# musaru/Fall_Multimodal

Measured on AMD Instinct MI355X. Metric: clips/sec (fwd+bwd) 3-stream Fall3, B=256, 1/2/4/8 GPUs; top-1 acc parity, higher is better.
Workload: dtype bf16x3; 1 GPU; fall3_3stream_coco_mmpose_V18_S6_B256_per_gpu; global_batch=256, seq_len=30, parallelism=dp1, joints=18, imu_axes=6, classes=11, hip_graph=False, ranks=1

## Files before the change

fall_multimodal_amd/_lib.py:

```python
from __future__ import annotations

import ctypes
import os

import torch

HERE = os.path.dirname(os.path.abspath(__file__))
LIB_PATH = os.environ.get("F3_LIB") or os.path.join(HERE, "libfall3.so")

EXPORTS = (
    "f3_net_create", "f3_net_destroy", "f3_net_num_entries", "f3_net_entry", "f3_net_param_count",
    "f3_net_buffer_count", "f3_net_counter_count", "f3_net_workspace_bytes", "f3_net_forward",
    "f3_net_loss", "f3_net_backward", "f3_rmsprop_step", "f3_conv_forward", "f3_status_string",
    "f3_net_debug_tensor", "f3_conv_backward_data", "f3_conv_backward_weight", "f3_conv_wgrad_packed", "f3_split_x3cat",
    "f3_conv_forward_x3cat", "f3_conv_backward_data_x3cat", "f3_conv_backward_weight_x3cat", "f3_conv_step_x3cat", "f3_graph_mix_forward",
    "f3_graph_mix_backward", "f3_graph_mix_forward_ex", "f3_graph_mix_backward_ex", "f3_gcn_dgrad_mix_x3",
    "f3_gcn_fwd_mix_x3",
    "f3_net_backward_phase",
    "f3_net_grad_split", "f3_net_wait_phase1", "f3_net_backward_rmsprop", "f3_net_fused_rmsprop", "f3_net_precision", "f3_net_status",
    "f3_targcn_create", "f3_targcn_destroy", "f3_targcn_num_entries", "f3_targcn_entry", "f3_targcn_param_count",
    "f3_targcn_buffer_count", "f3_targcn_workspace_bytes", "f3_targcn_forward", "f3_targcn_backward", "f3_targcn_stage_times", "f3_targcn_status", "f3_net_sensor_times", "f3_soft_ce",
    "f3_sktr_create", "f3_sktr_destroy", "f3_sktr_num_entries", "f3_sktr_entry", "f3_sktr_param_count",
    "f3_sktr_buffer_count", "f3_sktr_counter_count", "f3_sktr_workspace_bytes", "f3_sktr_forward", "f3_sktr_backward",
    "f3_musa_create", "f3_musa_destroy", "f3_musa_num_entries", "f3_musa_entry", "f3_musa_param_count",
    "f3_musa_buffer_count", "f3_musa_counter_count", "f3_musa_workspace_bytes", "f3_musa_forward", "f3_musa_backward",
    "f3_musa_guards",
    "f3_dwconv_t_forward", "f3_pointwise_conv", "f3_rgb_scratch_floats", "f3_rgb_forward", "f3_rgb_backward",
    "f3_optim_scalars_bytes", "f3_optim_step", "f3_optim_step_ranges", "f3_net_backward_optim", "f3_net_entry_nograd",
    "f3_metrics_bytes", "f3_metrics_reset", "f3_metrics_update", "f3_segment_norms_scratch_bytes", "f3_segment_norms",
    "f3_soft_ce_ex", "f3_net_loss_ex", "f3_grad_accumulate",
)

F3_OK, F3_EINVAL, F3_EBATCH, F3_EHIP, F3_ESTATE, F3_EDEVICE = 0, 1001, 1002, 1003, 1004, 1005
ENTRY_PARAM, ENTRY_BUFFER, ENTRY_COUNTER = 0, 1, 2
OPT_RMSPROP, OPT_SGD, OPT_ADAM, OPT_ADAMW = 0, 1, 2, 3
OPT_MAX_SKIP = 4
METRICS_MAXK, METRICS_MAXC = 8, 64


class F3OptimConfig(ctypes.Structure):
# ... 65 lines not shown
        "f3_metrics_update": (I, [P, P, P, P, P, I, I, ctypes.POINTER(I), I, P]),
        "f3_segment_norms_scratch_bytes": (I64, [I64, I]),
        "f3_segment_norms": (I, [P, P, P, I, P, P, I64, ctypes.c_double, P]),
        "f3_soft_ce_ex": (I, [P, P, P, I, I, F, P, P, P]),
        "f3_net_loss_ex": (I, [P, I, P, P, F, P, P, P]),
        "f3_grad_accumulate": (I, [P, P, I64, P, P]),
        "f3_conv_forward": (I, [P, P, P, P, P, I, I, I, I, I, I, I, I, I, P]),
        "f3_status_string": (ctypes.c_char_p, [I]),
        "f3_net_debug_tensor": (P, [P, I, P, I, I, ctypes.c_char_p]),
        "f3_conv_backward_data": (I, [P, P, P, P, I, I, I, I, I, I, I, I, I, P]),
        "f3_conv_backward_weight": (I, [P, P, P, P, I, I, I, I, I, I, I, I, I, P]),
        "f3_conv_wgrad_packed": (I, [P, P, P, ctypes.c_longlong, I, I, I, I, I, I, I, I, P]),
        "f3_split_x3cat": (I, [P, P, ctypes.c_int64, I, P]),
        "f3_conv_forward_x3cat": (I, [P, P, P, P, P, I, I, I, I, I, I, I, I, P]),
        "f3_conv_backward_data_x3cat": (I, [P, P, P, P, I, I, I, I, I, I, I, I, P]),
        "f3_conv_backward_weight_x3cat": (I, [P, P, P, P, I, I, I, I, I, I, I, I, P]),
        "f3_conv_step_x3cat": (I, [I, P, P, P, P, P, P, P, P, P, P, F, P, P, I, I, I, I, I, P]),
        "f3_graph_mix_forward": (I, [P, P, P, I, I, I, I, P]),
        "f3_graph_mix_backward": (I, [P, P, P, P, P, I, I, I, I, P]),
        "f3_graph_mix_forward_ex": (I, [P, P, P, I, I, I, I, I, P]),
        "f3_graph_mix_backward_ex": (I, [P, P, P, P, P, I, I, I, I, I, P]),
        "f3_gcn_dgrad_mix_x3": (I, [P, P, P, P, P, P, P, I, I, I, I, I, I, I, P]),
        "f3_gcn_fwd_mix_x3": (I, [P, P, P, P, P, P, P, P, P, I, I, I, I, I, P]),
        "f3_targcn_create": (I, [ctypes.POINTER(F3TargcnConfig), ctypes.POINTER(P)]),
        "f3_targcn_destroy": (None, [P]),
        "f3_targcn_num_entries": (I, [P]),
        "f3_targcn_entry": (I, [P, I, ctypes.POINTER(ctypes.c_char_p), ctypes.POINTER(I), ctypes.POINTER(I),
                                ctypes.POINTER(I64), ctypes.POINTER(I64)]),
        "f3_targcn_param_count": (I64, [P]),
        "f3_targcn_buffer_count": (I64, [P]),
        "f3_targcn_workspace_bytes": (I64, [P, I]),
        "f3_targcn_stage_times": (I, [P, I, P]),
        "f3_targcn_status": (I, [P, I]),
        "f3_net_sensor_times": (I, [P, I, P]),
        "f3_targcn_forward": (I, [P, I, P, P, P, P, P, P]),
        "f3_targcn_backward": (I, [P, I, P, P, P, P, P, P]),
        "f3_soft_ce": (I, [P, P, I, I, P, P, P]),
        "f3_sktr_create": (I, [ctypes.POINTER(F3SktrConfig), ctypes.POINTER(P)]),
        "f3_sktr_destroy": (None, [P]),
        "f3_sktr_num_entries": (I, [P]),
        "f3_sktr_entry": (I, [P, I, ctypes.POINTER(ctypes.c_char_p), ctypes.POINTER(I), ctypes.POINTER(I),
                              ctypes.POINTER(I64), ctypes.POINTER(I64)]),
        "f3_sktr_param_count": (I64, [P]),
        "f3_sktr_buffer_count": (I64, [P]),
        "f3_sktr_counter_count": (I64, [P]),
        "f3_sktr_workspace_bytes": (I64, [P, I]),
# ... 49 lines not shown
```

fall_multimodal_amd/csrc/gcn_fwd.hip:

```cpp
#include "igemm.h"
#include "layers.h"

#include <algorithm>
#include <cstdlib>
#include <type_traits>

namespace f3 {

constexpr int GF_THREADS = 512;
constexpr int GF_VMAX = 18, GF_K = 3, GF_CIN = 64, GF_KC = GF_K * GF_CIN;
constexpr int GF_BM = 32, GF_KS = 2 * GF_KC / 32;
constexpr int GF_XD = 7, GF_NXB = GF_XD + 1;
constexpr int GF_RING = GF_BM * GF_NXB;
constexpr int GF_ZP = GF_BM * 4 * GF_KC / 16 / GF_THREADS;

template <int WN>
struct GfLds {
  static constexpr int NT = 64 * WN;
  static constexpr int ABUF = GF_BM * GF_KC * 2 * 2;
  static constexpr int OTS = NT + 4;
  static constexpr int X_OFF = 2 * ABUF;
  static constexpr int OT_OFF = X_OFF + GF_RING * GF_CIN * 4;
  static constexpr int BV_OFF = OT_OFF + GF_BM * OTS * 4;
  static constexpr int RED_OFF = BV_OFF + GF_VMAX * NT * 4;
  static constexpr int BYTES = RED_OFF + 2 * 2 * NT * 4;
  static constexpr int PIECES = GF_BM * NT * 4 / 16 / GF_THREADS;
};

typedef __bf16 gf_bf16x4 __attribute__((ext_vector_type(4)));
typedef unsigned gf_u32x4 __attribute__((ext_vector_type(4)));

F3_DEV void gf_a_split(float t, __bf16& hi, __bf16& lo) {
  const float h = __uint_as_float(__float_as_uint(t) & 0xffff0000u);
  hi = __builtin_bit_cast(__bf16, (unsigned short)(__float_as_uint(h) >> 16));
  lo = (__bf16)(t - h);
}

F3_DEV float gf_atil(const float* A, int K, int V, int wk, int v) {
  if (wk >= K * V || v >= V) return 0.f;
  const int w = wk / K, k = wk - w * K;
  return A[(k * V + v) * V + w];
}

F3_DEV f32x4 gf_mfma_x3m(bf16x8 ah, bf16x8 al, bf16x8 bh, bf16x8 bl, f32x4 c) {
  c = mfma_bf16x(al, bh, c);
  c = mfma_bf16x(ah, bl, c);
  return mfma_bf16x(ah, bh, c);
}

template <int WN>
__global__ __launch_bounds__(GF_THREADS) void gcn_fwd_mix_x3_kernel(GcnFwdMixArgs a, int per_wg) {
  using L = GfLds<WN>;
  constexpr int NT = L::NT, OTS = L::OTS, KS = GF_KS, K = GF_K, CIN = GF_CIN, PIECES = L::PIECES;
  constexpr int OPS = 1 + GF_ZP + PIECES;
  constexpr int NSTEADY = GF_ZP + OPS * (GF_XD - 2);
  static_assert(L::BYTES <= 160 * 1024 && NSTEADY < 64 && GF_ZP * GF_THREADS * 16 == L::ABUF, "gcn_fwd LDS / vmcnt");
  static_assert((GF_RING & (GF_RING - 1)) == 0 && PIECES >= 1, "ring");
  extern __shared__ __attribute__((aligned(16))) char gf_smem[];
  char* img = gf_smem + L::OT_OFF;
  float* bv = reinterpret_cast<float*>(gf_smem + L::BV_OFF);
  float* red = reinterpret_cast<float*>(gf_smem + L::RED_OFF);
  const int tid = threadIdx.x, lane = tid & 63;
  const int wave = __builtin_amdgcn_readfirstlane(tid >> 6);
  const int wm = wave & 1, wj = wave >> 1;
  const int mt = wave & 3, nh = wave >> 2;
  const int fr = lane & 15, fg = lane >> 4;
  const int V = a.V, KV = K * V, M = a.frames * V;
  const int ntiles = (M + GF_BM - 1) / GF_BM;
  const int range = xcd_remap(blockIdx.x, gridDim.x);
  const int tile0 = range * per_wg, tile1 = min(ntiles, tile0 + per_wg);
  if (tile0 >= tile1) return;
// ... 254 lines not shown
```

fall_multimodal_amd/csrc/gemm_big.hip:

```cpp
#include "igemm.h"

#include <type_traits>

#ifndef F3_TILE_BATCH
#define F3_TILE_BATCH 1
#endif
#ifndef F3_PROBE
#define F3_PROBE 0
#endif

namespace f3 {

constexpr int BG_MT = 9, BG_NT = 2, BG_NST = 3;
constexpr int BG_WAVES = 8, BG_THREADS = 64 * BG_WAVES;

typedef __attribute__((address_space(3))) const char lds_cchar_t;
template <int WM, int WN, int WIN = 0>
struct BigCfg {
  static constexpr int BM = 16 * BG_MT * WM, BN = 16 * BG_NT * WN;
  static constexpr int NW = WM * WN;
  static constexpr int CPW = WIN == 144 && WM == 2 ? 2 : 1;
  static constexpr int NPA = (CPW * WIN + 7) / 8;
  static constexpr int NST = (WIN == 540 || (WIN == 144 && WM == 1)) ? 2 : BG_NST, LA = NST - 1;
  static constexpr int AP = WIN ? (WIN == 540 || WM == 1 ? 8 : 16) : BM / 8, BP = BN / 8, NP = AP + BP;
// ... 814 lines not shown
          continue;
        } else {
          if (issue && !(F3_PROBE & 2)) stage(JS, c + CS);
          F3_W1_READS
          F3_W1_MFMAS
        }
        if (LA == 2 && issue) wait_vm<DPS>();
        else wait_vm<0>();
        if (!(F3_PROBE & 8)) __builtin_amdgcn_s_barrier();
      }
    }
#undef F3_W1_READS
#undef F3_AREAD1
#undef F3_W1_MFMAS
    __syncthreads();
    auto none = [](int) { return -1; };
    if (F3_PROBE & 16) {
      if (lane == 0) a.out[blockIdx.x * NW + wave] = acc[0][0][0] + acc[BG_MT - 1][BG_NT - 1][3];
      return;
    }
    big_epilogue<EPI, WM, WN, WIN>(a, acc, smem, n0, clip0, nclip, MODE, wpar, 0, none);
}

}

using namespace f3;

static int big_win_rows(const ConvGemmArgs& a) {
  const ConvGeom& g = a.g;
  const int cb = a.x3n ? 32 : G_BK;
  if ((g.Nc % 128 && g.Nc != 64) || g.KT != 9 || 2 * g.P != g.KT - 1 || g.Kc % cb || g.T_out <= 0 || g.M % (g.T_out * g.V))
    return 0;
  int wf, of;
  if (g.S == 1) {
    if (g.T_in != g.T_out) return 0;
    wf = of = g.T_in;
  } else if (g.S == 2) {
    wf = g.transposed ? g.T_in : (g.T_in + 1) / 2;
    of = g.transposed ? (g.T_out + 1) / 2 : g.T_out;
  } else {
    return 0;
  }
  const int rows = (wf > of ? wf : of) * g.V;
  if (g.Nc == 64) return g.S == 1 && rows <= 540 ? 540 : 0;
  return rows <= 144 ? 144 : rows <= 270 ? 270 : 0;
}
// ... 90 lines not shown
  }
  F3_WCASE(EPI_BIAS | EPI_STATS | EPI_GAP)
  F3_WCASE(EPI_RELUMASK)
  F3_WCASE(EPI_BIAS)
  F3_WCASE(0)
#undef F3_WCASE
  return F3_EINVAL;
}

int f3_igemm_big(const ConvGemmArgs* args, int epi, hipStream_t s) {
  const ConvGemmArgs& a = *args;
  if (a.g.M <= 0) return F3_OK;
  if (!f3_igemm_big_ok(a)) return F3_EINVAL;
  const int wrows = big_win_rows(a);
  if (wrows) {
    const int r = wrows == 144 ? launch_win<144>(a, epi, s)
                  : wrows == 270 ? launch_win<270>(a, epi, s) : launch_win<540>(a, epi, s);
    if (r != F3_EINVAL) return r;
  }
  if (a.g.Nc == 64) return F3_EINVAL;
  if (a.g.Nc == 256) return a.x3n ? launch_big<1, 8, true>(a, epi, s) : launch_big<1, 8, false>(a, epi, s);
  return a.x3n ? launch_big<2, 4, true>(a, epi, s) : launch_big<2, 4, false>(a, epi, s);
}
```

fall_multimodal_amd/csrc/igemm.h:

```cpp
#pragma once
#include "common.h"
#include "kernels.h"

namespace f3 {

typedef __bf16 bf16x8 __attribute__((ext_vector_type(8)));
typedef __attribute__((address_space(3))) void lds_void_t;

constexpr int G_BK = 64;

F3_DEV f32x4 mfma_bf16x(bf16x8 a, bf16x8 b, f32x4 c) { return __builtin_amdgcn_mfma_f32_16x16x32_bf16(a, b, c, 0, 0, 0); }

F3_DEV int g_src_row(int n, int t, int v, int dt, const ConvGeom& g) {
  int ti;
  if (!g.transposed) {
    ti = t * g.S + dt - g.P;
    if (ti < 0 || ti >= g.T_in) return -1;
  } else {
    const int num = t + g.P - dt;
    if (num < 0 || (num % g.S) != 0) return -1;
    ti = num / g.S;
    if (ti >= g.T_in) return -1;
  }
  return (n * g.T_in + ti) * g.V + v;
}

F3_DEV int swz(int r, int c) { return c ^ (r & 7); }

F3_DEV int x3n_col(int C, int i0, int cg) { return i0 + 8 * cg + (cg >= 4 ? C - 32 : 0); }

__host__ __device__ inline bool igemm_parity(const ConvGeom& g) {
  return g.transposed && g.S == 2 && (g.KT == 1 || g.Kc >= 256);
}

// ... 34 lines not shown
```

fall_multimodal_amd/csrc/kernels.h:

```cpp
#pragma once
#include <hip/hip_runtime.h>
#include "common.h"

namespace f3 {

struct ConvGeom {
  int M;
  int Nc;
  int Kc;
  int KT, S, P;
  int transposed;
  int T_out, T_in, V;
  int lda, ldo;
};

enum : int {
  EPI_BIAS = 1,
  EPI_BIASV = 2,
  EPI_STATS = 4,
  EPI_GAP = 8,
  EPI_RELUMASK = 16,
  EPI_ADD = 32,
};

struct ConvGemmArgs {
  ConvGeom g;
  const float* in;
  const float* w;
  const unsigned short* wb;
  const unsigned short* inb;
  const unsigned short* zero;
  unsigned short* outb;
  float* out;
  BnRef pro_bn;
  const float* bias;
  double* st_sum;
  double* st_sq;
  float* gap;
  const float* aux;
  int ldaux;
  const unsigned short* auxb;
  BnRef epi_bn;
  int x3;
  int x3n;
};

enum : int { WG_OUT_CONV = 0, WG_OUT_GCN = 1 };

struct WgradArgs {
  ConvGeom g;
  const float* dy;
  int ldy;
  const float* in;
  float* dw;
  float* db;
  int outmap;
  int gcn_cin;
  BnRef pro_bn;
  int rows_per_split;
  int bf16;
  const unsigned short* dyb;
  const unsigned short* inb;
  const unsigned short* zero;
  int xcd;
  float* slab;
  long long slab_cap;
  float* dw_ref;
// ... 41 lines not shown
```

fall_multimodal_amd/csrc/layers.h:

```cpp
#pragma once
#include "common.h"

namespace f3 {

enum : int { PREP_MUL = 0, PREP_PACK_CONV, PREP_PACK_CONV_T, PREP_PACK_GCN, PREP_PACK_GCN_T, PREP_GCN_BIAS, PREP_COPY,
              PREP_UNPACK_CONV };

struct PrepJob {
  int type, n;
  float* dst;
  const float* s0;
  const float* s1;
  const float* s2;
  int d0, d1, d2;
  int bf16;
};

struct DataBnArgs {
  int N, T, V, C, motion;
  const float* skel;
  float* out;
  int act16;
  BnRef bn;
  double* st_sum;
// ... 196 lines not shown
struct PrepTable {
  int n;
  PrepJob jobs[kMaxPrepJobs];
};
constexpr int kMaxBnJobs = 56;
struct BnRunTable {
  int n;
  BnRunJob jobs[kMaxBnJobs];
};

}

int f3_prep(const f3::PrepTable& t, hipStream_t s);
int f3_databn_fwd(const f3::DataBnArgs* a, hipStream_t s);
int f3_databn_bwd(const f3::DataBnArgs* a, hipStream_t s);
int f3_mix_fwd(const f3::MixArgs* a, hipStream_t s);
int f3_mix_bwd(const f3::MixArgs* a, hipStream_t s);
int f3_mix_bwd_parts(const f3::MixArgs* a);
bool f3_gcn_dgrad_mix_ok(int K, int V, int Cin, int C);
int f3_gcn_dgrad_mix(const f3::GcnDgradMixArgs* a, hipStream_t s);
int f3_gcn_dgrad_mix_parts(const f3::GcnDgradMixArgs* a);
bool f3_gcn_fwd_mix_ok(int K, int V, int Cin, int C);
int f3_gcn_fwd_mix(const f3::GcnFwdMixArgs* a, hipStream_t s);
bool f3_mix_lds_ok(int K, int V, int Cin);
bool f3_mix_x3_ok(int K, int V, int Cin);
int f3_split_x3(const float* x, unsigned short* out, long long rows, int C, hipStream_t s);
int f3_gcn_bias_bwd(const f3::GcnBiasBwdArgs* a, hipStream_t s);
bool f3_gcn0_ok(int K, int V, int Ci, int C);
int f3_gcn0_fwd(const f3::Gcn0Args* a, hipStream_t s);
int f3_gcn0_bwd(const f3::Gcn0Args* a, hipStream_t s);
int f3_gcn0_bwd_parts(const f3::Gcn0Args* a);
int f3_databn_bwd2(const f3::DataBnArgs* a, hipStream_t s);
int f3_block_out(f3::BlockArgs a, hipStream_t s);
int f3_block_bwd_reduce(f3::BlockArgs a, hipStream_t s);
int f3_block_bwd_apply(f3::BlockArgs a, hipStream_t s);
int f3_bn_bwd_apply(f3::BnBwdArgs a, hipStream_t s);
int f3_bn_bwd_parts(int N, int TV, int V);
int f3_block_chunks(int TV);
int f3_bnrelu_bf16(const f3::BnReluArgs* a, hipStream_t s);
constexpr int kColsumJobs = 10;
struct ColsumJob {
  const float* part;
  float* out;
  long long ld;
  int rows, cols;
};
// ... 9 lines not shown
```

fall_multimodal_amd/csrc/net.cpp:

```cpp
#include <hip/hip_runtime.h>

#include <algorithm>
#include <cstdio>
#include <functional>
#include <cstdlib>
#include <cstring>
#include <string>
#include <vector>

#include "common.h"
#include "status_ring.h"
#include "kernels.h"
#include "layers.h"
#include "sensor.h"
#include "fall3.h"

using namespace f3;

namespace {

struct Entry {
  std::string name;
  int kind;
  std::vector<int64_t> shape;
// ... 469 lines not shown

void add_job(PrepTable& t, int type, int n, float* dst, const float* s0, const float* s1, const float* s2, int d0,
             int d1, int d2, int bf16 = 0) {
  PrepJob& j = t.jobs[t.n++];
  j.type = type; j.n = n; j.dst = dst; j.s0 = s0; j.s1 = s1; j.s2 = s2; j.d0 = d0; j.d1 = d1; j.d2 = d2;
  j.bf16 = bf16;
}

inline const unsigned short* bf(const float* p, int on) { return on ? reinterpret_cast<const unsigned short*>(p) : nullptr; }
inline int is_x3(const f3_net& n) { return n.cfg.precision == F3_PRECISION_BF16X3; }
inline int side_pct(bool split, int l) { return split && l >= 2 ? 75 : 0; }
constexpr int x3code() { return 4; }
inline int x3mul(int code) { return code == 4 ? 2 : 1; }
inline void x3_gemm(ConvGemmArgs& a, int C) {
  a.x3n = 1;
  a.g.lda = 2 * C;
}

inline bool gcn_dgrad_fused() {
  static const bool on = !getenv("F3_GCN_DGRAD_FUSED") || atoi(getenv("F3_GCN_DGRAD_FUSED")) != 0;
  return on;
}

inline bool gcn_fwd_fused() {
  static const bool on = !getenv("F3_GCN_FWD_FUSED") || atoi(getenv("F3_GCN_FWD_FUSED")) != 0;
  return on;
}

inline int wcode(const f3_net& n) { return n.cfg.precision == F3_PRECISION_BF16 ? 1 : is_x3(n) ? 2 : 0; }
inline unsigned short* bfa(float* p, int on) { return on ? reinterpret_cast<unsigned short*>(p) : nullptr; }

void add_bnrun(BnRunTable& t, const Ptrs& q, const BnIdx& bi, const double* sum, const double* sq, double count) {
  BnRunJob& j = t.jobs[t.n++];
  j.sum = sum; j.sumsq = sq; j.count = count; j.C = bi.C;
  j.rmean = q.b(bi.rm); j.rvar = q.b(bi.rv); j.nbt = q.c(bi.nbt);
}

int stream_forward_layer(const f3_net& net, int si, int N, int train, const Ptrs& q, Ws& w, BnRunTable& run,
                         hipStream_t s, int l);

int stream_forward(const f3_net& net, int si, int N, int train, const Ptrs& q, Ws& w, const float* skel,
                   BnRunTable& run, hipStream_t s, int stage) {
  if (stage >= 0) return stream_forward_layer(net, si, N, train, q, w, run, s, stage);
  const StreamIdx& S = net.st[si];
  StreamWs& W = w.st[si];
  const int K = net.K, V = net.V, eval = !train;
  const int hb = net.cfg.precision == F3_PRECISION_BF16;
  const int wc = wcode(net);
  PrepTable pt;
// ... 37 lines not shown
  StreamWs& W = w.st[si];
  const int K = net.K, V = net.V, eval = !train;
  const int hb = net.cfg.precision == F3_PRECISION_BF16;
  const int x3 = is_x3(net), wq = hb || x3;
  {
    const LayerIdx& L = S.L[l];
    LayerWs& X = W.L[l];
    const int C = L.cout, Ci = L.cin, Ti = L.T_in, To = L.T_out;
    const int Mi = N * Ti * V, Mo = N * To * V;
    const BnRef bn1 = q.ref(L.bn1, X.bn1, (float)Mi, eval);
    const BnRef bn2 = q.ref(L.bn2, X.bn2, (float)Mo, eval);
    BnRef bnr;
    std::memset(&bnr, 0, sizeof(bnr));
    if (L.res == RES_CONV) bnr = q.ref(L.bnr, X.bnr, (float)Mo, eval);
    if ((hb || x3) && f3_gcn0_ok(K, V, Ci, C)) {
      Gcn0Args g0;
      std::memset(&g0, 0, sizeof(g0));
      g0.frames = N * Ti; g0.K = K; g0.V = V; g0.Ci = Ci; g0.A = X.aeff;
      g0.x = reinterpret_cast<const unsigned short*>(X.x); g0.w = bf(X.gw, 1); g0.beff = X.beff;
      g0.z = bfa(X.z, 1); g0.g = bfa(X.g, 1); g0.st_sum = X.bn1.fsum; g0.st_sq = X.bn1.fsq;
      g0.f32 = x3;
      F3_TRY(f3_gcn0_fwd(&g0, s));
    } else if (x3 && f3_mix_x3_ok(K, V, Ci) && Ci == 64 && K * Ci == 192 && V <= 18 && (C == 64 || C == 128) &&
               gcn_fwd_fused() && f3_gcn_fwd_mix_ok(K, V, Ci, C)) {
      GcnFwdMixArgs gf;
      std::memset(&gf, 0, sizeof(gf));
      gf.frames = N * Ti; gf.K = K; gf.V = V; gf.Cin = Ci; gf.C = C; gf.A = X.aeff; gf.x = X.x;
      gf.z3 = bfa(X.z, 1); gf.w = bf(X.gw, 1); gf.bias = X.beff; gf.g = X.g;
      gf.st_sum = X.bn1.fsum; gf.st_sq = X.bn1.fsq; gf.zero = w.zero;
      F3_TRY(f3_gcn_fwd_mix(&gf, s));
    } else {
      MixArgs mx;
      std::memset(&mx, 0, sizeof(mx));
      mx.K = K; mx.V = V; mx.Cin = Ci; mx.frames = N * Ti; mx.A = X.aeff; mx.x = X.x; mx.z = X.z;
      mx.zb = bfa(X.z, hb); mx.x16 = hb; mx.x3 = x3;
      const bool gcat = x3 && f3_mix_x3_ok(K, V, Ci);
      mx.z3 = bfa(X.z, gcat);
      F3_TRY(f3_mix_fwd(&mx, s));
      ConvGemmArgs ga;
      std::memset(&ga, 0, sizeof(ga));
      ga.g = geom(Mi, C, K * Ci, 1, 1, 0, 0, Ti, Ti, V, K * Ci, C);
      ga.in = hb ? nullptr : X.z; ga.inb = bfa(X.z, hb); ga.zero = w.zero;
      ga.w = X.gw; ga.wb = bf(X.gw, wq); ga.out = X.g; ga.outb = bfa(X.g, hb); ga.x3 = x3;
      ga.bias = X.beff; ga.st_sum = X.bn1.fsum; ga.st_sq = X.bn1.fsq;
      if (gcat) {
        ga.x3 = 0; ga.in = nullptr; ga.inb = bfa(X.z, 1);
        x3_gemm(ga, K * Ci);
      }
      F3_TRY(f3_conv_gemm(&ga, 0, EPI_BIASV | EPI_STATS, s));
    }
    if (L.res == RES_CONV) {
      ConvGemmArgs ra;
      std::memset(&ra, 0, sizeof(ra));
// ... 1262 lines not shown
}

int f3_gcn_fwd_mix_x3(const float* A_eff, const float* x, const float* w, void* wpack, const float* bias_v, void* z3,
                      float* g, double* st_sum, double* st_sq, int frames, int K, int V, int Cin, int C,
                      void* stream) {
  hipStream_t s = (hipStream_t)stream;
  if (!A_eff || !x || !wpack || !bias_v || !z3 || !g || !st_sum || !st_sq || frames < 0) return F3_EINVAL;
  if (!f3_gcn_fwd_mix_ok(K, V, Cin, C)) return F3_EINVAL;
  if (w) {
    PrepTable t;
    t.n = 0;
    add_job(t, PREP_PACK_CONV, C * K * Cin * x3mul(x3code()), static_cast<float*>(wpack), w, nullptr, nullptr, C,
            K * Cin, 1, x3code());
    F3_TRY(f3_prep(t, s));
  }
  GcnFwdMixArgs a;
  std::memset(&a, 0, sizeof(a));
  a.frames = frames; a.K = K; a.V = V; a.Cin = Cin; a.C = C; a.A = A_eff; a.x = x;
  a.z3 = static_cast<unsigned short*>(z3); a.w = static_cast<const unsigned short*>(wpack); a.bias = bias_v; a.g = g;
  a.st_sum = st_sum; a.st_sq = st_sq; a.zero = test_zero_page();
  return f3_gcn_fwd_mix(&a, s);
}

void* f3_net_debug_tensor(f3_net* net, int batch, void* workspace, int stream, int layer, const char* what) {
  if (!net || stream < 0 || stream >= net->nstreams || layer < 0 || layer > 6) return nullptr;
  Ws w = plan(*net, batch, (char*)workspace);
  StreamWs& W = w.st[stream];
  LayerWs& X = W.L[layer];
  const std::string k(what);
  if (k == "x") return (void*)X.x;
  if (k == "z") return X.z;
  if (k == "g") return X.g;
  if (k == "h") return X.h;
  if (k == "r") return X.r;
  if (k == "out") return X.out;
  if (k == "att") return X.att;
  if (k == "dh") return X.dh;
  if (k == "u") return X.u;
  if (k == "dv") return W.dv;
  if (k == "dg") return X.dg;
  if (k == "dZ") return W.dZ;
  if (k == "dres") return X.dres;
  if (k == "dx0") return W.dx[0];
  if (k == "dx1") return W.dx[1];
  if (k == "bn1_fsum") return X.bn1.fsum;
  if (k == "bn1_fsq") return X.bn1.fsq;
// ... 37 lines not shown
```

include/fall3.h:

```cpp
#ifndef FALL3_H
#define FALL3_H
#include <stdint.h>

#ifdef __cplusplus
extern "C" {
#endif

#define F3_OK 0
#define F3_EINVAL 1001
#define F3_EBATCH 1002
#define F3_EHIP 1003
#define F3_ESTATE 1004
#define F3_EDEVICE 1005

enum { F3_MODEL_TWO_STGCAN_BILSTM = 0, F3_MODEL_TWO_STGCAN = 1, F3_MODEL_STGCN = 2, F3_MODEL_BILSTM = 3 };
enum { F3_SENSOR_NONE = 0, F3_SENSOR_BILSTM = 1, F3_SENSOR_CNN_BILSTM = 2 };
enum { F3_NAMING_PACKAGE = 0, F3_NAMING_NOTEBOOK = 1 };
enum { F3_PRECISION_FP32 = 0,
       F3_PRECISION_BF16 = 1,
       F3_PRECISION_BF16_FP32IN = 2,
       F3_PRECISION_BF16X3 = 4  };
enum { F3_ENTRY_PARAM = 0, F3_ENTRY_BUFFER = 1, F3_ENTRY_COUNTER = 2 };

typedef struct f3_config {
// ... 122 lines not shown
                      double* st_sq, int N, int T_in, int T_out, int V, int Cin, int Cout, int stride, int transposed,
                      int epi, void* stream);

long long f3_rgb_scratch_floats(int B, int T);
int f3_rgb_forward(const void* frames, const void* wpack, const float* bias, float* feat, int B, int T, void* stream);
int f3_rgb_backward(const void* frames, const void* wpack, const float* bias, const float* dfeat, float* dw, float* db,
                    float* scratch, long long scratch_floats, int B, int T, void* stream);

int f3_graph_mix_forward(const float* A_eff, const float* x, float* z, int frames, int K, int V, int Cin,
                         void* stream);
int f3_graph_mix_backward(const float* A_eff, const float* x, const float* dz, float* dx, float* dA, int frames, int K,
                          int V, int Cin, void* stream);
enum { F3_MIX_X_BF16 = 1, F3_MIX_Z_BF16 = 2, F3_MIX_X3 = 4, F3_MIX_Z3 = 8 };
int f3_graph_mix_forward_ex(const float* A_eff, const void* x, void* z, int frames, int K, int V, int Cin, int flags,
                            void* stream);
int f3_graph_mix_backward_ex(const float* A_eff, const void* x, const void* dz, float* dx, float* dA, int frames, int K,
                             int V, int Cin, int flags, void* stream);
int f3_gcn_dgrad_mix_x3(const void* dg3, const float* w, void* wpack, const float* A_eff, const float* x, float* dx,
                        float* dA, int frames, int K, int V, int Cin, int C, int accumulate, int max_workgroups,
                        void* stream);
int f3_gcn_fwd_mix_x3(const float* A_eff, const float* x, const float* w, void* wpack, const float* bias_v, void* z3,
                      float* g, double* st_sum, double* st_sq, int frames, int K, int V, int Cin, int C,
                      void* stream);

const char* f3_status_string(int status);

typedef struct f3_targcn_config {
  int num_node;
  int num_class;
  int precision;
} f3_targcn_config;

typedef struct f3_targcn f3_targcn;

int f3_targcn_create(const f3_targcn_config* cfg, f3_targcn** out);
void f3_targcn_destroy(f3_targcn* net);
int f3_targcn_num_entries(const f3_targcn* net);
int f3_targcn_entry(const f3_targcn* net, int i, const char** name, int* kind, int* ndim, int64_t* shape8,
                    int64_t* offset);
int64_t f3_targcn_param_count(const f3_targcn* net);
int64_t f3_targcn_buffer_count(const f3_targcn* net);
int64_t f3_targcn_workspace_bytes(const f3_targcn* net, int batch);
int f3_targcn_forward(f3_targcn* net, int batch, const float* params, const float* buffers, const float* source,
                      float* out, void* workspace, void* stream);
int f3_targcn_backward(f3_targcn* net, int batch, const float* params, const float* buffers, const float* dout,
                       float* grads, void* workspace, void* stream);
// ... 62 lines not shown
```

Measured before the change: 33540 clips/s.

## Fuse graph mixing into big GEMM kernel for wide GCN forward layers

Adds a fused kernel that computes the adjacency mixing (x times A, bf16x3 split) inside the large igemm tile loop. Mixed z values are written to LDS and fed to the GEMM, with the z3 copy also stored to global for backward. This covers layers with Cin 128/256 and C 128/256, removing the separate mix kernel launch and its z round trip through global memory before the GEMM. It is enabled by default through fused level 2, and it adds register and LDS pressure plus tricky interleaving of mix and GEMM stages.

```diff
diff --git a/fall_multimodal_amd/_lib.py b/fall_multimodal_amd/_lib.py
--- a/fall_multimodal_amd/_lib.py
+++ b/fall_multimodal_amd/_lib.py
@@ -16,6 +16,7 @@
     "f3_conv_forward_x3cat", "f3_conv_backward_data_x3cat", "f3_conv_backward_weight_x3cat", "f3_conv_step_x3cat", "f3_graph_mix_forward",
     "f3_graph_mix_backward", "f3_graph_mix_forward_ex", "f3_graph_mix_backward_ex", "f3_gcn_dgrad_mix_x3",
     "f3_gcn_fwd_mix_x3",
+    "f3_gcn_fwd_mix_big_x3",
     "f3_net_backward_phase",
     "f3_net_grad_split", "f3_net_wait_phase1", "f3_net_backward_rmsprop", "f3_net_fused_rmsprop", "f3_net_precision", "f3_net_status",
     "f3_targcn_create", "f3_targcn_destroy", "f3_targcn_num_entries", "f3_targcn_entry", "f3_targcn_param_count",
@@ -127,6 +128,7 @@
         "f3_graph_mix_backward_ex": (I, [P, P, P, P, P, I, I, I, I, I, P]),
         "f3_gcn_dgrad_mix_x3": (I, [P, P, P, P, P, P, P, I, I, I, I, I, I, I, P]),
         "f3_gcn_fwd_mix_x3": (I, [P, P, P, P, P, P, P, P, P, I, I, I, I, I, P]),
+        "f3_gcn_fwd_mix_big_x3": (I, [P, P, P, P, P, P, P, P, P, I, I, I, I, I, P]),
         "f3_targcn_create": (I, [ctypes.POINTER(F3TargcnConfig), ctypes.POINTER(P)]),
         "f3_targcn_destroy": (None, [P]),
         "f3_targcn_num_entries": (I, [P]),
diff --git a/fall_multimodal_amd/csrc/gcn_fwd.hip b/fall_multimodal_amd/csrc/gcn_fwd.hip
--- a/fall_multimodal_amd/csrc/gcn_fwd.hip
+++ b/fall_multimodal_amd/csrc/gcn_fwd.hip
@@ -27,26 +27,7 @@
   static constexpr int PIECES = GF_BM * NT * 4 / 16 / GF_THREADS;
 };
 
-typedef __bf16 gf_bf16x4 __attribute__((ext_vector_type(4)));
 typedef unsigned gf_u32x4 __attribute__((ext_vector_type(4)));
-
-F3_DEV void gf_a_split(float t, __bf16& hi, __bf16& lo) {
-  const float h = __uint_as_float(__float_as_uint(t) & 0xffff0000u);
-  hi = __builtin_bit_cast(__bf16, (unsigned short)(__float_as_uint(h) >> 16));
-  lo = (__bf16)(t - h);
-}
-
-F3_DEV float gf_atil(const float* A, int K, int V, int wk, int v) {
-  if (wk >= K * V || v >= V) return 0.f;
-  const int w = wk / K, k = wk - w * K;
-  return A[(k * V + v) * V + w];
-}
-
-F3_DEV f32x4 gf_mfma_x3m(bf16x8 ah, bf16x8 al, bf16x8 bh, bf16x8 bl, f32x4 c) {
-  c = mfma_bf16x(al, bh, c);
-  c = mfma_bf16x(ah, bl, c);
-  return mfma_bf16x(ah, bh, c);
-}
 
 template <int WN>
 __global__ __launch_bounds__(GF_THREADS) void gcn_fwd_mix_x3_kernel(GcnFwdMixArgs a, int per_wg) {
diff --git a/fall_multimodal_amd/csrc/gemm_big.hip b/fall_multimodal_amd/csrc/gemm_big.hip
--- a/fall_multimodal_amd/csrc/gemm_big.hip
+++ b/fall_multimodal_amd/csrc/gemm_big.hip
@@ -1,5 +1,7 @@
 #include "igemm.h"
-
+#include "layers.h"
+
+#include <cstring>
 #include <type_traits>
 
 #ifndef F3_TILE_BATCH
@@ -860,6 +862,285 @@
     big_epilogue<EPI, WM, WN, WIN>(a, acc, smem, n0, clip0, nclip, MODE, wpar, 0, none);
 }
 
+constexpr int BX_V = 18, BX_K = 3;
+typedef unsigned u32x2_t __attribute__((ext_vector_type(2)));
+
+F3_DEV float lds_rd32(unsigned addr) {
+  float v;
+  asm volatile("ds_read_b32 %0, %1" : "=v"(v) : "v"(addr));
+  return v;
+}
+F3_DEV void pin_f(float& v) { asm volatile("" : "+v"(v)); }
+F3_DEV void lds_wr64(unsigned addr, u32x2_t v) { asm volatile("ds_write_b64 %0, %1" ::"v"(addr), "v"(v) : "memory"); }
+
+template <int FPW>
+struct MixLane {
+  unsigned xrd;
+  unsigned estep;
+  unsigned wr[FPW];
+  unsigned zrd[FPW];
+  int zoff[FPW];
+  int zrow8;
+  bool vall, v01, wok1, z2;
+};
+
+F3_DEV __attribute__((always_inline)) void mixa_load_tap(unsigned tab, int fr, int fg, bf16x8 (&bh)[2], bf16x8 (&bl)[2]) {
+  float t[2][8];
+#pragma unroll
+  for (int q = 0; q < 2; ++q)
+#pragma unroll
+    for (int e = 0; e < 8; ++e)
+      t[q][e] = lds_rd32(tab + (min(8 * fg + e, BX_V - 1) * BX_V + min(16 * q + fr, BX_V - 1)) * 4);
+  asm volatile("s_waitcnt lgkmcnt(0)"
+               : "+v"(t[0][0]), "+v"(t[0][1]), "+v"(t[0][2]), "+v"(t[0][3]), "+v"(t[0][4]), "+v"(t[0][5]), "+v"(t[0][6]),
+                 "+v"(t[0][7]), "+v"(t[1][0]), "+v"(t[1][1]), "+v"(t[1][2]), "+v"(t[1][3]), "+v"(t[1][4]), "+v"(t[1][5]),
+                 "+v"(t[1][6]), "+v"(t[1][7])
+               :
+               : "memory");
+#pragma unroll
+  for (int q = 0; q < 2; ++q)
+#pragma unroll
+    for (int e = 0; e < 8; ++e) {
+      __bf16 h, l;
+      gf_a_split(8 * fg + e < BX_V && 16 * q + fr < BX_V ? t[q][e] : 0.f, h, l);
+      bh[q][e] = h;
+      bl[q][e] = l;
+    }
+}
+
+template <int WM, int WN, int FPW, bool MIX, bool GEMM>
+F3_DEV __attribute__((always_inline)) void mix_gemm_step(unsigned sl, const MixLane<FPW>& L, const bf16x8 (&mbh)[2],
+                                                         const bf16x8 (&mbl)[2], char* zdst, unsigned l0, int wm, int wn,
+                                                         int fr, int fg, f32x4 (&acc)[BG_MT][BG_NT]) {
+  static_assert(BG_NT == 2 && BG_MT == 9, "batched tile reads");
+  constexpr int AP = BigCfg<WM, WN>::AP, NF = BG_NT + BG_MT;
+  const int ra = wm * 144 + fr, rw = wn * 32 + fr;
+  const unsigned ah[2] = {l0 + ra * 128 + swz(ra, fg) * 16, l0 + ra * 128 + swz(ra, 4 + fg) * 16};
+  const unsigned bh[2] = {l0 + AP * 1024 + rw * 128 + swz(rw, fg) * 16, l0 + AP * 1024 + rw * 128 + swz(rw, 4 + fg) * 16};
+  float xv[2][8];
+  u32x4_t f[2][NF];
+  f32x4 macc[FPW][2][2];
+  auto frag_reads = [&](auto ksc) {
+    constexpr int ks = decltype(ksc)::value;
+    f[ks][0] = lds_rd128(bh[ks]);
+    f[ks][1] = lds_rd128o<2048>(bh[ks]);
+    static_for<0, BG_MT>([&](auto x) { f[ks][BG_NT + decltype(x)::value] = lds_rd128o<2048 * decltype(x)::value>(ah[ks]); });
+  };
+  auto products = [&](auto ksc) {
+    constexpr int ks = decltype(ksc)::value;
+#pragma unroll
+    for (int qq = 0; qq < NF; ++qq) pin_v(f[ks][qq]);
+#pragma unroll
+    for (int x = 0; x < BG_MT; ++x)
+#pragma unroll
+      for (int y = 0; y < BG_NT; ++y) {
+        acc[x][y] = mfma_bf16x(__builtin_bit_cast(bf16x8, f[ks][BG_NT + x]), __builtin_bit_cast(bf16x8, f[0][y]), acc[x][y]);
+        if (ks == 1)
+          acc[x][y] = mfma_bf16x(__builtin_bit_cast(bf16x8, f[0][BG_NT + x]), __builtin_bit_cast(bf16x8, f[1][y]), acc[x][y]);
+      }
+#pragma unroll
+    for (int x = 0; x < BG_MT; ++x)
+#pragma unroll
+      for (int y = 0; y < BG_NT; ++y) pin_v(acc[x][y]);
+  };
+  auto x_reads = [&](int j) {
+#pragma unroll
+    for (int mt = 0; mt < 2; ++mt)
+#pragma unroll
+      for (int e = 0; e < 8; ++e)
+        xv[mt][e] = lds_rd32(sl + (L.xrd ^ (unsigned)(mt << 6)) + j * (BX_V * 128) + (e == 0 ? 0u : 128u + (e - 1) * L.estep));
+  };
+  auto z_writes = [&](int j) {
+#pragma unroll
+    for (int mt = 0; mt < 2; ++mt)
+#pragma unroll
+      for (int q = 0; q < 2; ++q) {
+        gf_bf16x4 h, l;
+#pragma unroll
+        for (int e = 0; e < 4; ++e) {
+          h[e] = (__bf16)macc[j][mt][q][e];
+          l[e] = (__bf16)(macc[j][mt][q][e] - (float)h[e]);
+        }
+        if (q == 0 || L.wok1) {
+          const unsigned ad = sl + (L.wr[j] ^ (unsigned)(mt << 5)) + q * 2048;
+          lds_wr64(ad, __builtin_bit_cast(u32x2_t, h));
+          lds_wr64(ad ^ 64u, __builtin_bit_cast(u32x2_t, l));
+        }
+      }
+  };
+  if constexpr (MIX) x_reads(0);
+  if constexpr (GEMM) frag_reads(std::integral_constant<int, 0>{});
+  if constexpr (MIX) {
+#pragma unroll
+    for (int j = 0; j < FPW; ++j) {
+      if (j > 0) x_reads(j);
+      if (GEMM && j == 0) wait_lgkm<NF>();
+      else wait_lgkm<0>();
+      bf16x8 xah[2], xal[2];
+#pragma unroll
+      for (int mt = 0; mt < 2; ++mt)
+#pragma unroll
+        for (int e = 0; e < 8; ++e) {
+          pin_f(xv[mt][e]);
+          const float x = (e < 2 ? L.v01 : L.vall) ? xv[mt][e] : 0.f;
+          const __bf16 h = (__bf16)x;
+          xah[mt][e] = h;
+          xal[mt][e] = (__bf16)(x - (float)h);
+        }
+#pragma unroll
+      for (int mt = 0; mt < 2; ++mt)
+#pragma unroll
+        for (int q = 0; q < 2; ++q)
+          macc[j][mt][q] = gf_mfma_x3m(xah[mt], xal[mt], mbh[q], mbl[q], f32x4{0.f, 0.f, 0.f, 0.f});
+      if constexpr (!GEMM) z_writes(j);
+    }
+#pragma unroll
+    for (int j = 0; j < FPW; ++j)
+#pragma unroll
+      for (int mt = 0; mt < 2; ++mt)
+#pragma unroll
+        for (int q = 0; q < 2; ++q) pin_v(macc[j][mt][q]);
+  }
+  if constexpr (GEMM) {
+    wait_lgkm<0>();
+    products(std::integral_constant<int, 0>{});
+  }
+  if constexpr (MIX && GEMM) {
+#pragma unroll
+    for (int j = 0; j < FPW; ++j) z_writes(j);
+  }
+  if constexpr (GEMM) {
+    frag_reads(std::integral_constant<int, 1>{});
+    wait_lgkm<0>();
+    products(std::integral_constant<int, 1>{});
+  }
+  if constexpr (MIX) {
+    u32x4_t z[FPW][3];
+#pragma unroll
+    for (int j = 0; j < FPW; ++j)
+#pragma unroll
+      for (int i = 0; i < 3; ++i) z[j][i] = lds_rd128(sl + L.zrd[j] + 1024 * i);
+    wait_lgkm<0>();
+#pragma unroll
+    for (int j = 0; j < FPW; ++j)
+#pragma unroll
+      for (int i = 0; i < 3; ++i) {
+        pin_v(z[j][i]);
+        if (L.zoff[j] >= 0 && (i < 2 || L.z2)) *reinterpret_cast<u32x4_t*>(zdst + L.zoff[j] + i * L.zrow8) = z[j][i];
+      }
+  }
+}
+
+template <int WM, int WN>
+__global__ __launch_bounds__(BG_THREADS) void igemm_big_mix(ConvGemmArgs a) {
+  using Cfg = BigCfg<WM, WN>;
+  constexpr int EPI = EPI_BIASV | EPI_STATS;
+  constexpr int BM = Cfg::BM, AP = Cfg::AP, BP = Cfg::BP, STAGE = Cfg::STAGE;
+  constexpr int V = BX_V, NF = BM / V, FPW = NF / BG_WAVES;
+  constexpr int XW = (AP + BG_WAVES - 1) / BG_WAVES, BW = BP / BG_WAVES, ZS = 3 * FPW;
+  static_assert(WM * WN == BG_WAVES && NF * V == BM && FPW * BG_WAVES == NF && BW * BG_WAVES == BP, "whole frames per wave");
+  static_assert(STAGE % 1024 == 0 && BW + ZS < 64, "stage alignment (XORed offsets), vmcnt");
+  constexpr int SMEM = Cfg::EPI_OFF + BX_K * V * V * 4 > Cfg::SMEM ? Cfg::EPI_OFF + BX_K * V * V * 4 : Cfg::SMEM;
+  static_assert(SMEM <= 160 * 1024, "LDS");
+  __shared__ __attribute__((aligned(1024))) char smem[SMEM];
+  const ConvGeom& g = a.g;
+  const int tid = threadIdx.x, lane = tid & 63;
+  const int wave = __builtin_amdgcn_readfirstlane(tid >> 6);
+  const int wm = wave / WN, wn = wave % WN, fr = lane & 15, fg = lane >> 4;
+  const int m0 = xcd_remap(blockIdx.x, gridDim.x) * BM;
+  const int M = g.M, Cin = g.Kc / BX_K, kpt = Cin / 32, nstep = BX_K * kpt;
+  const int rowB = 4 * g.Kc;
+  const bool part = m0 + BM > M;
+  auto phys = [&](int r) -> int { return r < M ? r : -1; };
+
+  const int sub = lane >> 3, pch = lane & 7;
+  const char* xsrc[XW];
+  int xadv[XW];
+#pragma unroll
+  for (int i = 0; i < XW; ++i) {
+    const int R = ((wave + BG_WAVES * i) % AP) * 8 + sub, m = m0 + R, v = R % V;
+    const bool ok = m < M;
+    xsrc[i] = ok ? reinterpret_cast<const char*>(a.in + (size_t)m * Cin) + ((pch ^ (((v >> 3) & 1) << 2)) << 4)
+                 : reinterpret_cast<const char*>(a.zero);
+    xadv[i] = ok ? 128 : 0;
+  }
+  const char* bsrc[BW];
+#pragma unroll
+  for (int i = 0; i < BW; ++i) {
+    const int j = (wave + BG_WAVES * i) * 8 + sub;
+    bsrc[i] = reinterpret_cast<const char*>(a.wb + (size_t)j * (2 * g.Kc) + swz(j, pch) * 8);
+  }
+  auto stage = [&](int t, int cb, int buf) {
+    char* sb = smem + buf * STAGE;
+#pragma unroll
+    for (int i = 0; i < XW; ++i) {
+      const void* src = xsrc[i] + cb * xadv[i];
+      __builtin_amdgcn_global_load_lds(src, (lds_void_t*)(sb + ((wave + BG_WAVES * i) % AP) * 1024), 16, 0, 0);
+    }
+#pragma unroll
+    for (int i = 0; i < BW; ++i) {
+      const void* src = bsrc[i] + t * 128;
+      __builtin_amdgcn_global_load_lds(src, (lds_void_t*)(sb + (AP + wave + BG_WAVES * i) * 1024), 16, 0, 0);
+    }
+  };
+  stage(0, 0, 0);
+  stage(1, 1, 1);
+
+  MixLane<FPW> L;
+  L.xrd = (wave * FPW * V + 8 * min(fg, 2)) * 128 + (((fr >> 2) ^ (fg == 1 ? 4 : 0)) << 4) + (fr & 3) * 4;
+  L.estep = fg < 2 ? 128u : 0u;
+  L.vall = fg < 2;
+  L.v01 = fg < 3;
+  L.wok1 = 16 + fr < V;
+  L.z2 = lane + 128 < 8 * V;
+  L.zrow8 = 8 * rowB;
+#pragma unroll
+  for (int j = 0; j < FPW; ++j) {
+    const int R0 = (wave * FPW + j) * V;
+    L.wr[j] = (R0 + fr) * 128 + (((fg >> 1) ^ ((R0 + fr) & 7)) << 4) + (fg & 1) * 8;
+    {
+      const int R = R0 + (lane >> 3), c = lane & 7;
+      L.zrd[j] = R * 128 + ((c ^ (R & 7)) << 4);
+      L.zoff[j] = m0 + R0 < M ? R * rowB + (c >> 2) * (rowB / 2) + (c & 3) * 16 : -1;
+    }
+  }
+  for (int i = tid; i < BX_K * V * V; i += BG_THREADS) reinterpret_cast<float*>(smem + Cfg::EPI_OFF)[i] = a.mix_A[i];
+  f32x4 acc[BG_MT][BG_NT];
+#pragma unroll
+  for (int x = 0; x < BG_MT; ++x)
+#pragma unroll
+    for (int y = 0; y < BG_NT; ++y) acc[x][y] = f32x4{0.f, 0.f, 0.f, 0.f};
+  wait_vm<0>();
+  wait_lgkm<0>();
+  __builtin_amdgcn_s_barrier();
+
+  const unsigned lds0 = (unsigned)(size_t)(lds_cchar_t*)smem;
+  char* zt = reinterpret_cast<char*>(a.mix_z) + (size_t)m0 * rowB;
+  bf16x8 mbh[2], mbl[2];
+  int u = 0;
+  for (int k = 0; k < BX_K; ++k) {
+    mixa_load_tap(lds0 + Cfg::EPI_OFF + k * V * V * 4, fr, fg, mbh, mbl);
+    for (int cb = 0; cb < kpt; ++cb, ++u) {
+      if (u >= 1 && u + 1 < nstep) stage(u + 1, cb + 1 == kpt ? 0 : cb + 1, (u + 1) % 3);
+      const unsigned sl = lds0 + (u % 3) * STAGE, l0 = lds0 + ((u + 2) % 3) * STAGE;
+      char* zdst = zt + (k * Cin + cb * 32) * 2;
+      if (u >= 1) {
+        mix_gemm_step<WM, WN, FPW, true, true>(sl, L, mbh, mbl, zdst, l0, wm, wn, fr, fg, acc);
+      } else {
+        mix_gemm_step<WM, WN, FPW, true, false>(sl, L, mbh, mbl, zdst, 0u, wm, wn, fr, fg, acc);
+        if (u >= 1) mix_gemm_step<WM, WN, FPW, false, true>(0u, L, mbh, mbl, zdst, l0, wm, wn, fr, fg, acc);
+      }
+      if (part || u + 1 >= nstep) wait_vm<0>();
+      else wait_vm<BW + ZS>();
+      wait_lgkm<0>();
+      __builtin_amdgcn_s_barrier();
+    }
+  }
+  mix_gemm_step<WM, WN, FPW, false, true>(0u, L, mbh, mbl, zt, lds0 + ((nstep - 1) % 3) * STAGE, wm, wn, fr, fg, acc);
+  __syncthreads();
+  big_epilogue<EPI, WM, WN, 0>(a, acc, smem, 0, 0, 0, 0, 0, m0, phys);
+}
+
 }
 
 using namespace f3;
@@ -996,3 +1277,32 @@
   if (a.g.Nc == 256) return a.x3n ? launch_big<1, 8, true>(a, epi, s) : launch_big<1, 8, false>(a, epi, s);
   return a.x3n ? launch_big<2, 4, true>(a, epi, s) : launch_big<2, 4, false>(a, epi, s);
 }
+
+bool f3_gcn_fwd_mix_big_ok(int K, int V, int Cin, int C) {
+  return K == BX_K && V == BX_V && ((Cin == 128 && (C == 128 || C == 256)) || (Cin == 256 && C == 256));
+}
+
+int f3_gcn_fwd_mix_big(const GcnFwdMixArgs* args, hipStream_t s) {
+  const GcnFwdMixArgs& m = *args;
+  if (!f3_gcn_fwd_mix_big_ok(m.K, m.V, m.Cin, m.C) || m.frames < 0) return F3_EINVAL;
+  if (!m.A || !m.x || !m.z3 || !m.w || !m.bias || !m.g || !m.st_sum || !m.st_sq || !m.zero) return F3_EINVAL;
+  if ((long long)m.frames * m.V >= (1ll << 31) - 2 * 288) return F3_EINVAL;
+  if ((reinterpret_cast<uintptr_t>(m.x) | reinterpret_cast<uintptr_t>(m.z3) | reinterpret_cast<uintptr_t>(m.w)) & 15)
+    return F3_EINVAL;
+  if (m.frames == 0) return F3_OK;
+  ConvGemmArgs a;
+  std::memset(&a, 0, sizeof(a));
+  a.g.M = m.frames * m.V; a.g.Nc = m.C; a.g.Kc = m.K * m.Cin; a.g.KT = 1; a.g.S = 1; a.g.P = 0; a.g.transposed = 0;
+  a.g.T_out = a.g.T_in = 1; a.g.V = m.V; a.g.lda = 2 * m.K * m.Cin; a.g.ldo = m.C;
+  a.in = m.x; a.wb = m.w; a.zero = m.zero; a.out = m.g; a.bias = m.bias; a.st_sum = m.st_sum; a.st_sq = m.st_sq;
+  a.x3n = 1; a.mix_A = m.A; a.mix_z = m.z3;
+  if (m.C == 256) {
+    const int tiles = (a.g.M + BigCfg<1, 8>::BM - 1) / BigCfg<1, 8>::BM;
+    hipLaunchKernelGGL((igemm_big_mix<1, 8>), dim3(tiles), dim3(BG_THREADS), 0, s, a);
+  } else {
+    const int tiles = (a.g.M + BigCfg<2, 4>::BM - 1) / BigCfg<2, 4>::BM;
+    hipLaunchKernelGGL((igemm_big_mix<2, 4>), dim3(tiles), dim3(BG_THREADS), 0, s, a);
+  }
+  F3_LAUNCH_CHECK();
+  return F3_OK;
+}
diff --git a/fall_multimodal_amd/csrc/igemm.h b/fall_multimodal_amd/csrc/igemm.h
--- a/fall_multimodal_amd/csrc/igemm.h
+++ b/fall_multimodal_amd/csrc/igemm.h
@@ -10,6 +10,26 @@
 constexpr int G_BK = 64;
 
 F3_DEV f32x4 mfma_bf16x(bf16x8 a, bf16x8 b, f32x4 c) { return __builtin_amdgcn_mfma_f32_16x16x32_bf16(a, b, c, 0, 0, 0); }
+
+typedef __bf16 gf_bf16x4 __attribute__((ext_vector_type(4)));
+
+F3_DEV void gf_a_split(float t, __bf16& hi, __bf16& lo) {
+  const float h = __uint_as_float(__float_as_uint(t) & 0xffff0000u);
+  hi = __builtin_bit_cast(__bf16, (unsigned short)(__float_as_uint(h) >> 16));
+  lo = (__bf16)(t - h);
+}
+
+F3_DEV float gf_atil(const float* A, int K, int V, int wk, int v) {
+  if (wk >= K * V || v >= V) return 0.f;
+  const int w = wk / K, k = wk - w * K;
+  return A[(k * V + v) * V + w];
+}
+
+F3_DEV f32x4 gf_mfma_x3m(bf16x8 ah, bf16x8 al, bf16x8 bh, bf16x8 bl, f32x4 c) {
+  c = mfma_bf16x(al, bh, c);
+  c = mfma_bf16x(ah, bl, c);
+  return mfma_bf16x(ah, bh, c);
+}
 
 F3_DEV int g_src_row(int n, int t, int v, int dt, const ConvGeom& g) {
   int ti;
diff --git a/fall_multimodal_amd/csrc/kernels.h b/fall_multimodal_amd/csrc/kernels.h
--- a/fall_multimodal_amd/csrc/kernels.h
+++ b/fall_multimodal_amd/csrc/kernels.h
@@ -43,6 +43,8 @@
   BnRef epi_bn;
   int x3;
   int x3n;
+  const float* mix_A;
+  unsigned short* mix_z;
 };
 
 enum : int { WG_OUT_CONV = 0, WG_OUT_GCN = 1 };
diff --git a/fall_multimodal_amd/csrc/layers.h b/fall_multimodal_amd/csrc/layers.h
--- a/fall_multimodal_amd/csrc/layers.h
+++ b/fall_multimodal_amd/csrc/layers.h
@@ -242,6 +242,8 @@
 int f3_gcn_dgrad_mix_parts(const f3::GcnDgradMixArgs* a);
 bool f3_gcn_fwd_mix_ok(int K, int V, int Cin, int C);
 int f3_gcn_fwd_mix(const f3::GcnFwdMixArgs* a, hipStream_t s);
+bool f3_gcn_fwd_mix_big_ok(int K, int V, int Cin, int C);
+int f3_gcn_fwd_mix_big(const f3::GcnFwdMixArgs* a, hipStream_t s);
 bool f3_mix_lds_ok(int K, int V, int Cin);
 bool f3_mix_x3_ok(int K, int V, int Cin);
 int f3_split_x3(const float* x, unsigned short* out, long long rows, int C, hipStream_t s);
diff --git a/fall_multimodal_amd/csrc/net.cpp b/fall_multimodal_amd/csrc/net.cpp
--- a/fall_multimodal_amd/csrc/net.cpp
+++ b/fall_multimodal_amd/csrc/net.cpp
@@ -515,9 +515,9 @@
   return on;
 }
 
-inline bool gcn_fwd_fused() {
-  static const bool on = !getenv("F3_GCN_FWD_FUSED") || atoi(getenv("F3_GCN_FWD_FUSED")) != 0;
-  return on;
+inline int gcn_fwd_fused() {
+  static const int level = !getenv("F3_GCN_FWD_FUSED") ? 2 : atoi(getenv("F3_GCN_FWD_FUSED"));
+  return level;
 }
 
 inline int wcode(const f3_net& n) { return n.cfg.precision == F3_PRECISION_BF16 ? 1 : is_x3(n) ? 2 : 0; }
@@ -601,13 +601,20 @@
       g0.f32 = x3;
       F3_TRY(f3_gcn0_fwd(&g0, s));
     } else if (x3 && f3_mix_x3_ok(K, V, Ci) && Ci == 64 && K * Ci == 192 && V <= 18 && (C == 64 || C == 128) &&
-               gcn_fwd_fused() && f3_gcn_fwd_mix_ok(K, V, Ci, C)) {
+               gcn_fwd_fused() >= 1 && f3_gcn_fwd_mix_ok(K, V, Ci, C)) {
       GcnFwdMixArgs gf;
       std::memset(&gf, 0, sizeof(gf));
       gf.frames = N * Ti; gf.K = K; gf.V = V; gf.Cin = Ci; gf.C = C; gf.A = X.aeff; gf.x = X.x;
       gf.z3 = bfa(X.z, 1); gf.w = bf(X.gw, 1); gf.bias = X.beff; gf.g = X.g;
       gf.st_sum = X.bn1.fsum; gf.st_sq = X.bn1.fsq; gf.zero = w.zero;
       F3_TRY(f3_gcn_fwd_mix(&gf, s));
+    } else if (x3 && f3_mix_x3_ok(K, V, Ci) && gcn_fwd_fused() >= 2 && f3_gcn_fwd_mix_big_ok(K, V, Ci, C)) {
+      GcnFwdMixArgs gf;
+      std::memset(&gf, 0, sizeof(gf));
+      gf.frames = N * Ti; gf.K = K; gf.V = V; gf.Cin = Ci; gf.C = C; gf.A = X.aeff; gf.x = X.x;
+      gf.z3 = bfa(X.z, 1); gf.w = bf(X.gw, 1); gf.bias = X.beff; gf.g = X.g;
+      gf.st_sum = X.bn1.fsum; gf.st_sq = X.bn1.fsq; gf.zero = w.zero;
+      F3_TRY(f3_gcn_fwd_mix_big(&gf, s));
     } else {
       MixArgs mx;
       std::memset(&mx, 0, sizeof(mx));
@@ -1916,6 +1923,27 @@
   return f3_gcn_fwd_mix(&a, s);
 }
 
+int f3_gcn_fwd_mix_big_x3(const float* A_eff, const float* x, const float* w, void* wpack, const float* bias_v,
+                          void* z3, float* g, double* st_sum, double* st_sq, int frames, int K, int V, int Cin, int C,
+                          void* stream) {
+  hipStream_t s = (hipStream_t)stream;
+  if (!A_eff || !x || !wpack || !bias_v || !z3 || !g || !st_sum || !st_sq || frames < 0) return F3_EINVAL;
+  if (!f3_gcn_fwd_mix_big_ok(K, V, Cin, C)) return F3_EINVAL;
+  if (w) {
+    PrepTable t;
+    t.n = 0;
+    add_job(t, PREP_PACK_CONV, C * K * Cin * x3mul(x3code()), static_cast<float*>(wpack), w, nullptr, nullptr, C,
+            K * Cin, 1, x3code());
+    F3_TRY(f3_prep(t, s));
+  }
+  GcnFwdMixArgs a;
+  std::memset(&a, 0, sizeof(a));
+  a.frames = frames; a.K = K; a.V = V; a.Cin = Cin; a.C = C; a.A = A_eff; a.x = x;
+  a.z3 = static_cast<unsigned short*>(z3); a.w = static_cast<const unsigned short*>(wpack); a.bias = bias_v; a.g = g;
+  a.st_sum = st_sum; a.st_sq = st_sq; a.zero = test_zero_page();
+  return f3_gcn_fwd_mix_big(&a, s);
+}
+
 void* f3_net_debug_tensor(f3_net* net, int batch, void* workspace, int stream, int layer, const char* what) {
   if (!net || stream < 0 || stream >= net->nstreams || layer < 0 || layer > 6) return nullptr;
   Ws w = plan(*net, batch, (char*)workspace);
diff --git a/include/fall3.h b/include/fall3.h
--- a/include/fall3.h
+++ b/include/fall3.h
@@ -168,6 +168,9 @@
 int f3_gcn_fwd_mix_x3(const float* A_eff, const float* x, const float* w, void* wpack, const float* bias_v, void* z3,
                       float* g, double* st_sum, double* st_sq, int frames, int K, int V, int Cin, int C,
                       void* stream);
+int f3_gcn_fwd_mix_big_x3(const float* A_eff, const float* x, const float* w, void* wpack, const float* bias_v,
+                          void* z3, float* g, double* st_sum, double* st_sq, int frames, int K, int V, int Cin, int C,
+                          void* stream);
 
 const char* f3_status_string(int status);
 
```

New measurement: 33740 clips/s (median of 6 runs). About the same (+0.6%).
